# OpenPPL/ppl.llm.serving

Measured on AMD Instinct MI355X. Metric: decode tokens/sec, LLaMA-7B int8 (W8A16), max-running-batch 1024, higher is better.
Workload: dtype fp16 activations, int8 weights (W8A16), int8-g8 KV, fp32 accumulate

## Files before the change

ppl.llm.serving_amd/csrc/k_gemm.hip:

```cpp
#include <stdarg.h>
#include <stdio.h>
#include <stdlib.h>

#include <algorithm>

#include <type_traits>
#include "k_gemm_dev.h"

namespace pplhip {

void LinearRoute::add(const char* fmt, ...) {
    if (!buf || cap <= 0 || len >= cap - 1) return;
    if (len > 0) buf[len++] = ' ';
    va_list ap;
    va_start(ap, fmt);
    const int n = vsnprintf(buf + len, (size_t)(cap - len), fmt, ap);
    va_end(ap);
    len = n < 0 ? len : (len + n < cap - 1 ? len + n : cap - 1);
    buf[len] = 0;
}

template <int WQ, int EPI>
__global__ __launch_bounds__(256) void gemm_kernel(const uint16_t* __restrict__ x, const void* __restrict__ wv,
                                                   const uint16_t* __restrict__ scale, int64_t M, int N, int K, int group,
// ... 595 lines not shown

template <class F>
void for_each_half128(F&& f) {
    f(int_c<3>{}, int_c<16>{}); f(int_c<3>{}, int_c<32>{}); f(int_c<2>{}, int_c<64>{}); f(int_c<3>{}, int_c<64>{});
    f(int_c<3>{}, int_c<80>{}); f(int_c<3>{}, int_c<96>{}); f(int_c<3>{}, int_c<112>{}); f(int_c<3>{}, int_c<128>{});
}
void run_w8_half128(const LinearPart& p, const LinearArgs& a) {
    static LdsOptIn once;
    if (once.first())
        for_each_epi([](auto E) {
            for_each_half128([&](auto ST, auto BM) { set_max_lds(half128_lds_bytes(ST, BM), gemm_w8_half128_kernel<E, ST, BM>); });
        });
    dispatch_epi(p.epi, [&](auto E) {
        for_each_half128([&](auto ST, auto BM) {
            if (ST == p.stages && BM == p.bm)
                hipLaunchKernelGGL((gemm_w8_half128_kernel<E, ST, BM>), dim3(p.grid_x, p.grid_y), dim3(p.threads), p.lds, a.s, a.x, (const int8_t*)a.w,
                                   a.scale, p.M, a.N, a.K, a.y, a.ldy, p.n_tiles, p.kt_per, a.ws);
        });
    });
}

void run_ring(const LinearPart& p, const LinearArgs& a) {
    dispatch_int<8, 4, 0>(p.wq, [&](auto WQ) {
        dispatch_epi(p.epi, [&](auto E) {
            dispatch_int<2, 3, 4>(p.stages, [&](auto ST) {
                auto go = [&](auto kernel) {
                    hipLaunchKernelGGL(kernel, dim3(p.grid_x, p.grid_y), dim3(p.threads), 0, a.s, a.x, a.w, a.scale, p.M, a.N, a.K, a.y, a.ldy, p.n_tiles,
                                       p.m_tiles, map_pack(p.map), p.kt_per, a.ws);
                };
                if constexpr (WQ == 8 && ST >= 3) {
                    if (p.wl == 6) return go(gemm_dma_kernel<WQ, E, ST, 6>);
                }
                if (p.wl == 5) go(gemm_dma_kernel<WQ, E, ST, 5>);
                else if (p.bm == 64) go(gemm_dma_kernel<WQ, E, ST, 1, 64>);
                else if (p.maxg == 16) go(gemm_dma_kernel<WQ, E, ST, 1, G_BM, 16>);
                else go(gemm_dma_kernel<WQ, E, ST, 1>);
            });
        });
    });
}

void run_generic(const LinearPart& p, const LinearArgs& a) {
    dispatch_int<0, 8, 4>(p.wq, [&](auto WQ) {
        dispatch_epi(p.epi, [&](auto E) {
            hipLaunchKernelGGL((gemm_kernel<WQ, E>), dim3(p.grid_x), dim3(p.threads), 0, a.s, a.x, a.w, a.scale, p.M, a.N, a.K, a.group, a.y, a.ldy,
                               p.n_tiles, p.m_tiles);
        });
    });
}

}

hipError_t launch_linear(hipStream_t s, const uint16_t* x, const void* w, const uint16_t* scale, int wq_bit, int group,
                         int64_t M, int N, int K, void* y, int64_t ldy, bool out_fp32, float* ws, size_t ws_bytes, bool swiglu, SplitSlabs* defer,
                         LinearRoute* route) {
    if (defer) *defer = SplitSlabs{};
    if (M == 0) return hipSuccess;
    if (swiglu && out_fp32) return hipErrorInvalidValue;
    LinearProblem pr;
    pr.wq_bit = wq_bit, pr.group = group, pr.M = M, pr.N = N, pr.K = K, pr.ldy = ldy;
    pr.epi = swiglu ? EPI_SWIGLU : (out_fp32 ? EPI_F32 : EPI_F16);
    pr.ws_bytes = ws ? ws_bytes : 0;
    pr.accept_defer = defer != nullptr;
    pr.x = (uintptr_t)x, pr.w = (uintptr_t)w, pr.scale = (uintptr_t)scale, pr.y = (uintptr_t)y;
    if (!linear_problem_valid(pr)) return hipErrorInvalidValue;
    static const LinearTuning tuning = LinearTuning::from_env();
    const LinearPlan plan = plan_linear(pr, tuning);
    if (!plan.ok) return hipErrorInvalidValue;
    if (route) {
        char text[512];
        format_route(plan, text, (int)sizeof text);
        route->add("%s", text);
        if (route->dry) return hipSuccess;
    }
    const uint16_t* rscale = wq_bit == 8 ? scale : nullptr;
    for (int i = 0; i < plan.n_parts; ++i) {
        const LinearPart& p = plan.part[i];
        const LinearArgs a{s, x + p.m0 * K, w, scale, group, N, K, (char*)y + (size_t)p.m0 * ldy * (out_fp32 ? 4 : 2), ldy, ws};
        hipError_t e = hipSuccess;
        bool sub = false;
        switch (p.family) {
            case LF_GEMV_STREAM: sub = true, e = launch_gemv_stream(s, a.x, w, scale, wq_bit, group, p.M, N, K, a.y, ldy, p.epi); break;
            case LF_W4_PC: sub = true, e = launch_linear_w4_pc(s, a.x, w, scale, p.M, N, K, a.y, ldy, p.epi); break;
            case LF_W8_WIDE: sub = true, e = launch_linear_w8_wide(s, a.x, (const int8_t*)w, scale, p.M, N, K, a.y, ldy, p.epi, p.nc); break;
            case LF_GEMV: run_gemv(p, a); break;
            case LF_W8_256: run_w8_256(p, a); break;
            case LF_W8_HALF128: run_w8_half128(p, a); break;
            case LF_RING: run_ring(p, a); break;
            case LF_GENERIC: run_generic(p, a); break;
        }
        if (!sub) e = hipGetLastError();
        if (e != hipSuccess) return e;
        if (p.reduce == LR_DEFERRED) *defer = SplitSlabs{ws, p.splits, rscale, N, p.M};
        else if (p.reduce == LR_KERNEL && (e = launch_splitk_reduce(s, ws, p.splits, p.M, N, rscale, a.y, ldy, p.epi)) != hipSuccess) return e;
    }
    return hipSuccess;
}

}
```

ppl.llm.serving_amd/csrc/k_gemm_wide.hip:

```cpp
#include <stdlib.h>
#include "k_gemm_dev.h"

namespace pplhip {

namespace {

constexpr int WD_XP = WD_XB / 1024;

template <int EPI, int ST, int NC, int ABL = 0>
__global__ __launch_bounds__((NC + WD_NP) * 64) void gemm_w8_wide_kernel(const uint16_t* __restrict__ x, const int8_t* __restrict__ w,
                                                                  const uint16_t* __restrict__ scale, int64_t M, int N, int K,
                                                                  void* __restrict__ yv, int64_t ldy, int n_tiles, int m_tiles) {
    constexpr int WD_BN = 32 * NC, WD_NC = NC;
    constexpr int WD_WB = WD_BN * G_BK, WD_WP = WD_WB / 1024;
    constexpr int WD_PP = (WD_XP + WD_WP + WD_NP - 1) / WD_NP;
    extern __shared__ __attribute__((aligned(16))) char smem_wd[];
    char* const Xs0 = smem_wd;
    char* const Wq0 = smem_wd + ST * WD_XB;

    int nt, mt;
    xcd_tile((int)blockIdx.x, m_tiles, nt, mt);
    if (nt >= n_tiles) return;
    const int n0 = nt * WD_BN;
    const int64_t m0 = (int64_t)mt * WD_BM;

    const int tid = threadIdx.x, lane = tid & 63, wave = __builtin_amdgcn_readfirstlane(tid >> 6);
    const int ktiles = K / G_BK;
    constexpr int D = ST - 1;

    if (wave >= WD_NC) {
        const int pw = wave - WD_NC;
        const char* psrc[WD_PP];
        uint32_t pdst[WD_PP];
        const uint32_t xbase = lds_addr(Xs0), wbase = lds_addr(Wq0);
        const int npc = (WD_XP + WD_WP - pw + WD_NP - 1) / WD_NP;
#pragma unroll
        for (int j = 0; j < WD_PP; ++j) {
            const int P = pw + WD_NP * j;
            if (j < WD_XP / WD_NP) {
                const int p = P * 64 + lane, row = p >> 3, pos = (p & 7) ^ ((row >> 1) & 7);
                const int c = ((pos & 3) << 1) | (pos >> 2);
                int64_t m = m0 + row;
                if (m >= M) m = M - 1;
                psrc[j] = reinterpret_cast<const char*>(x + m * K + c * 8);
                pdst[j] = __builtin_amdgcn_readfirstlane(xbase + P * 1024);
            } else {
                const int Pw = (P < WD_XP + WD_WP ? P : WD_XP) - WD_XP;
                const int p = Pw * 64 + lane, row = p >> 2, c = (p & 3) ^ w_swz(row);
                int n = n0 + row;
                if (n >= N) n = N - 1;
                psrc[j] = reinterpret_cast<const char*>(w) + (int64_t)n * K + c * 16;
                pdst[j] = __builtin_amdgcn_readfirstlane(wbase + Pw * 1024);
            }
        }
#define WD_PRODUCE(KT, STG)                                                                                                          \
    do {                                                                                                                             \
        _Pragma("unroll") for (int j = 0; j < WD_PP; ++j)                                                                            \
            if (j < npc)                                                                                                             \
            glds16(psrc[j] + (int64_t)(KT) * (j < WD_XP / WD_NP ? G_BK * 2 : G_BK), pdst[j] + (STG) * (j < WD_XP / WD_NP ? WD_XB : WD_WB)); \
    } while (0)
#pragma unroll
        for (int d = 0; d < D; ++d)
            if (d < ktiles) WD_PRODUCE(d, d);
        int stn = D % ST;
        for (int t = 0; t < ktiles; ++t) {
            const int younger = (ktiles - 1 - t) < (D - 1) ? (ktiles - 1 - t) : (D - 1);
            if (younger >= 2) {
                if (npc == WD_PP) asm volatile("s_waitcnt vmcnt(%0)" ::"n"(2 * WD_PP) : "memory");
                else asm volatile("s_waitcnt vmcnt(%0)" ::"n"(2 * WD_PP - 2) : "memory");
            } else if (younger == 1) {
                if (npc == WD_PP) asm volatile("s_waitcnt vmcnt(%0)" ::"n"(WD_PP) : "memory");
                else asm volatile("s_waitcnt vmcnt(%0)" ::"n"(WD_PP - 1) : "memory");
            } else {
                asm volatile("s_waitcnt vmcnt(0)" ::: "memory");
            }
            if (!(ABL & 8)) __syncthreads();
            if (t + D < ktiles && !(ABL & 1)) WD_PRODUCE(t + D, stn);
            stn = stn == ST - 1 ? 0 : stn + 1;
        }
#undef WD_PRODUCE
        return;
    }

    const int l15 = lane & 15, kq = lane >> 4;
    const int nb = wave * 32;
    f4 acc[2][8];
#pragma unroll
    for (int i = 0; i < 2; ++i)
#pragma unroll
        for (int j = 0; j < 8; ++j) acc[i][j] = f4{0.f, 0.f, 0.f, 0.f};
    int st = 0;
    for (int t = 0; t < ktiles; ++t) {
        if (!(ABL & 8)) __syncthreads();
        const uint16_t* xs = reinterpret_cast<const uint16_t*>(Xs0 + st * WD_XB);
        const char* wq = Wq0 + st * WD_WB;
        st = st == ST - 1 ? 0 : st + 1;
        uint4 wraw[2];
#pragma unroll
        for (int i = 0; i < 2; ++i) {
            const int row = nb + i * 16 + l15;
            wraw[i] = *reinterpret_cast<const uint4*>(&wq[row * G_BK + (kq ^ w_swz(row)) * 16]);
        }
#pragma unroll
        for (int ks = 0; ks < 2; ++ks) {
            h8 a[2], bfr[8];
#pragma unroll
            for (int i = 0; i < 2; ++i) {
                if constexpr (ABL & 2) a[i] = __builtin_bit_cast(h8, make_uint4(wraw[i].x, wraw[i].y, wraw[i].z ^ ks, wraw[i].w));
                else a[i] = cvt_i8x8_f16(ks == 0 ? make_uint2(wraw[i].x, wraw[i].y) : make_uint2(wraw[i].z, wraw[i].w));
            }
#pragma unroll
            for (int j = 0; j < 8; ++j) {
                const int row = j * 16 + l15;
                bfr[j] = __builtin_bit_cast(h8, *reinterpret_cast<const uint4*>(&xs[((ABL & 4) ? 0 : row * G_BK) + g_swz(row, ks * 4 + kq) * 8]));
            }
#pragma unroll
            for (int i = 0; i < 2; ++i)
#pragma unroll
                for (int j = 0; j < 8; ++j) acc[i][j] = __builtin_amdgcn_mfma_f32_16x16x32_f16(a[i], bfr[j], acc[i][j], 0, 0, 0);
        }
    }

#pragma unroll
    for (int i = 0; i < 2; ++i) {
        const int n = n0 + nb + i * 16 + kq * 4;
        if (n >= N) continue;
        const h4 sh = __builtin_bit_cast(h4, *reinterpret_cast<const uint2*>(scale + n));
#pragma unroll
        for (int j = 0; j < 8; ++j) {
            const int64_t m = m0 + j * 16 + l15;
            if (m >= M) continue;
            store4<EPI>(yv, ldy, m, n, acc[i][j][0] * (float)sh[0], acc[i][j][1] * (float)sh[1], acc[i][j][2] * (float)sh[2],
                        acc[i][j][3] * (float)sh[3]);
        }
    }
}

}

hipError_t launch_linear_w8_wide(hipStream_t s, const uint16_t* x, const int8_t* w, const uint16_t* scale, int64_t M, int N, int K, void* y,
                                 int64_t ldy, int epi, int nc, LinearRoute* route) {
    LinearPart p;
    if (!plan_w8_wide(M, N, epi, nc, &p)) return hipErrorInvalidValue;
    if (route_part(route, p)) return hipSuccess;
    constexpr int ST = WD_ST;
    const size_t lds = p.lds;
    const int n_tiles = p.n_tiles, m_tiles = p.m_tiles;
    static LdsOptIn once;
    if (once.first()) for_each_epi([&](auto E) { set_max_lds(lds, gemm_w8_wide_kernel<E, ST, 12>); });
    dim3 grid(p.grid_x);
#ifdef WD_ABLATE_BUILD
    static const int abl = getenv("PPLHIP_GEMM_WIDE_ABLATE") ? atoi(getenv("PPLHIP_GEMM_WIDE_ABLATE")) : 0;
    bool ablated = true;
    dispatch_int<1, 2, 3, 4, 6, 7, 8, 15, 0>(abl, [&](auto A) {
        if constexpr (A == 0) ablated = false;
        else {
            set_max_lds(lds, gemm_w8_wide_kernel<EPI_F16, ST, 12, A>);
            hipLaunchKernelGGL((gemm_w8_wide_kernel<EPI_F16, ST, 12, A>), grid, dim3((12 + WD_NP) * 64), lds, s, x, w, scale, M, N, K, y, ldy, n_tiles, m_tiles);
        }
    });
    if (ablated) return hipGetLastError();
#endif
    dispatch_epi(epi, [&](auto E) {
        hipLaunchKernelGGL((gemm_w8_wide_kernel<E, ST, 12>), grid, dim3((12 + WD_NP) * 64), lds, s, x, w, scale, M, N, K, y, ldy, n_tiles, m_tiles);
    });
    return hipGetLastError();
}

}
```

ppl.llm.serving_amd/csrc/kernels.h:

```cpp
#pragma once
#include <hip/hip_runtime.h>
#include <stdint.h>
#include "k_common.h"
#include "linear_plan.h"

namespace pplhip {

struct SplitSlabs {
    const float* ws = nullptr;
    int splits = 0;
    const uint16_t* scale = nullptr;
    int N = 0;
    int64_t M = 0;
};
struct LinearRoute {
    char* buf = nullptr;
    int cap = 0;
    int len = 0;
    bool dry = false;
    void add(const char* fmt, ...) __attribute__((format(printf, 2, 3)));
};
#ifdef __HIPCC__
__device__ __forceinline__ void slab_load8(const SplitSlabs& sl, int64_t m, int n, float* o) {
    const float* p = sl.ws + m * sl.N + n;
    const int64_t zs = sl.M * sl.N;
    float4 c[8], d[8];
#pragma unroll
    for (int z = 0; z < 8; ++z) {
        const float* q = p + (z < sl.splits ? z : 0) * zs;
        c[z] = *reinterpret_cast<const float4*>(q);
        d[z] = *reinterpret_cast<const float4*>(q + 4);
    }
    float4 a = c[0], b = d[0];
#pragma unroll
    for (int z = 1; z < 8; ++z) {
        if (z < sl.splits) {
            a.x += c[z].x; a.y += c[z].y; a.z += c[z].z; a.w += c[z].w;
            b.x += d[z].x; b.y += d[z].y; b.z += d[z].z; b.w += d[z].w;
        }
    }
    if (sl.scale) {
        const h8 sh = __builtin_bit_cast(h8, *reinterpret_cast<const uint4*>(sl.scale + n));
        a.x *= (float)sh[0]; a.y *= (float)sh[1]; a.z *= (float)sh[2]; a.w *= (float)sh[3];
        b.x *= (float)sh[4]; b.y *= (float)sh[5]; b.z *= (float)sh[6]; b.w *= (float)sh[7];
    }
    o[0] = round_h(a.x); o[1] = round_h(a.y); o[2] = round_h(a.z); o[3] = round_h(a.w);
    o[4] = round_h(b.x); o[5] = round_h(b.y); o[6] = round_h(b.z); o[7] = round_h(b.w);
}
#endif

hipError_t launch_embedding(hipStream_t s, const int64_t* token_ids, const uint16_t* table, int64_t T, int hidden,
                            uint16_t* out);
hipError_t launch_rmsnorm(hipStream_t s, const uint16_t* x, const uint16_t* skip, const uint16_t* w, float eps,
                          int64_t rows, int hidden, const int64_t* gather_seq_starts, uint16_t* out,
                          uint16_t* residual_out, int8_t* qout = nullptr, float* sx = nullptr,
                          const SplitSlabs* skip_slabs = nullptr,
                          bool q_fp8 = false);
struct RmsnormForm {
    int maxc = 0, nt = 0;
};
hipError_t rmsnorm_form(int64_t rows, int hidden, int wide_max_rows, RmsnormForm* f);
int rmsnorm_wide_max_rows();
hipError_t launch_silu_mul(hipStream_t s, const uint16_t* gate_up, int64_t T, int inter, uint16_t* out);
hipError_t launch_gather_last_rows(hipStream_t s, const uint16_t* x, const int64_t* seq_starts, int64_t B, int hidden, uint16_t* out);

hipError_t launch_rope_kv_write(hipStream_t s, uint16_t* qkv, const float* cos_sin, const KvAddr& kv, int kv_fmt,
                                const int64_t* seq_starts, const int64_t* start_pos,
                                const int64_t* cache_indices, int64_t max_pages, int64_t B, int64_t t0, int64_t T, int H,
                                int Hkv, int D, const SplitSlabs* qkv_slabs = nullptr);

size_t attn_decode_workspace_bytes(int64_t nb, int H, int D, int split);
hipError_t launch_attn_decode(hipStream_t s, const uint16_t* qkv, const KvAddr& kv, int kv_fmt,
                              const int64_t* seq_starts, const int64_t* start_pos, const int64_t* cache_indices,
                              int64_t max_pages, int64_t nb, int H, int Hkv, int D, int64_t max_kv_len, int split,
                              int threads, float* workspace, uint16_t* out, hipEvent_t t0 = nullptr, hipEvent_t t1 = nullptr);
hipError_t launch_attn_reduce(hipStream_t s, const float* ws, int nsplit, int64_t n_row_heads, int D, uint16_t* out);

hipError_t launch_attn_prefill(hipStream_t s, const uint16_t* qkv, const KvAddr& kv, int kv_fmt,
                               const int64_t* seq_starts, const int64_t* start_pos, const int64_t* cache_indices,
                               int64_t max_pages, int64_t b0, int64_t B, int H, int Hkv, int D, int64_t max_seq_len,
                               uint16_t* out, int64_t max_kv_len = 0, float* ws = nullptr, size_t ws_bytes = 0, int64_t row0 = 0,
                               int64_t nrows = 0);

hipError_t launch_attn_prefill32(hipStream_t s, const uint16_t* qkv, const KvAddr& kv, int kv_fmt, const int64_t* seq_starts,
                                 const int64_t* start_pos, const int64_t* cache_indices, int64_t max_pages, int64_t b0, int64_t B,
                                 int H, int Hkv, int D, int64_t max_seq_len, uint16_t* out, int64_t max_kv_len = 0, float* ws = nullptr,
                                 size_t ws_bytes = 0, int64_t row0 = 0, int64_t nrows = 0);

bool attn_decode_gqa_supported(int kv_fmt, int H, int Hkv, int D);
hipError_t launch_attn_decode_gqa(hipStream_t s, const uint16_t* qkv, const KvAddr& kv, int kv_fmt,
                                  const int64_t* seq_starts, const int64_t* start_pos, const int64_t* cache_indices,
                                  int64_t max_pages, int64_t nb, int H, int Hkv, int D, int split, float* workspace,
                                  uint16_t* out, hipEvent_t t0 = nullptr, hipEvent_t t1 = nullptr);

hipError_t launch_linear_w8_wide(hipStream_t s, const uint16_t* x, const int8_t* w, const uint16_t* scale, int64_t M, int N, int K, void* y,
                                 int64_t ldy, int epi, int nc, LinearRoute* route = nullptr);
hipError_t launch_linear_w4_pc(hipStream_t s, const uint16_t* x, const void* w, const uint16_t* scale, int64_t M, int N, int K, void* y,
                               int64_t ldy, int epi, LinearRoute* route = nullptr);
hipError_t launch_linear(hipStream_t s, const uint16_t* x, const void* w, const uint16_t* scale, int wq_bit, int group,
                         int64_t M, int N, int K, void* y, int64_t ldy, bool out_fp32, float* ws = nullptr, size_t ws_bytes = 0,
                         bool swiglu = false, SplitSlabs* defer = nullptr,
                         LinearRoute* route = nullptr);
hipError_t launch_splitk_reduce(hipStream_t s, const float* ws, int splits, int64_t M, int N, const uint16_t* scale, void* y, int64_t ldy, int epi);
hipError_t launch_gemv_stream(hipStream_t s, const uint16_t* x, const void* w, const uint16_t* scale, int wq_bit, int group, int64_t M, int N,
                              int K, void* y, int64_t ldy, int epi, LinearRoute* route = nullptr);
hipError_t launch_quant_act(hipStream_t s, const uint16_t* x, int64_t M, int K, int64_t ldx, int8_t* q, int64_t ldq, float* sx);
hipError_t launch_quant_weight(hipStream_t s, const uint16_t* w, int N, int K, int8_t* q, int64_t ldq, uint16_t* scale);
hipError_t launch_linear_i8(hipStream_t s, const int8_t* xq, const float* sx, const int8_t* w, const uint16_t* scale, int64_t M, int N,
                            int K, void* y, int64_t ldy, bool out_fp32, bool swiglu);
hipError_t launch_quant_act_f8(hipStream_t s, const uint16_t* x, int64_t M, int K, int64_t ldx, uint8_t* q, int64_t ldq, float* sx);
hipError_t launch_quant_weight_f8(hipStream_t s, const uint16_t* w, int N, int K, uint8_t* q, int64_t ldq, uint16_t* scale);
hipError_t launch_linear_f8(hipStream_t s, const uint8_t* xq, const float* sx, const uint8_t* w, const uint16_t* scale, int64_t M, int N,
                            int K, void* y, int64_t ldy, bool out_fp32, bool swiglu);
hipError_t launch_interleave_rows(hipStream_t s, const void* src, void* dst, int rows, int64_t row_bytes);

constexpr int LORA_MAX_SLOTS = 64, LORA_MAX_RANK = 128;
struct LoraTile {
    int32_t slot;
    int32_t n;
    int32_t row[16];
};
struct LoraSlot {
    const uint16_t* a;
    const uint16_t* b;
    int32_t rp;
    float scale;
};
hipError_t launch_lora(hipStream_t s, const LoraTile* tiles, int ntiles, const LoraSlot* slots, const uint16_t* x, int64_t ldx, uint16_t* y,
                       int64_t ldy, int N, int K, uint16_t* t);

constexpr int P2P_MAX_RANKS = 8;
constexpr int P2P_MAX_BLOCKS = 64;
constexpr size_t P2P_FLAGS_START = 0;
constexpr size_t P2P_FLAGS_MID = (size_t)P2P_MAX_BLOCKS * P2P_MAX_RANKS * 4;
constexpr int P2P_CHANNELS = 2;
constexpr size_t P2P_CHANNEL_FLAG_BYTES = (size_t)2 * P2P_MAX_BLOCKS * P2P_MAX_RANKS * 4;
constexpr size_t P2P_DATA_START = 8192;
static_assert(P2P_CHANNELS * P2P_CHANNEL_FLAG_BYTES <= P2P_DATA_START, "flag words of every channel in front of the data");
constexpr uint32_t P2P_FLAG_REFRESH_EPOCHS = 1u << 30;
struct P2pPeers {
    char* base[P2P_MAX_RANKS];
};
hipError_t launch_p2p_flag_refresh(hipStream_t s, char* my_base, int channel, uint32_t epoch);
hipError_t launch_p2p_allreduce(hipStream_t s, const P2pPeers& peers, int me, int n, size_t data_off, size_t scratch_off, int64_t count,
                                uint32_t epoch, uint64_t timeout_ticks, uint32_t* status, int channel = 0);
constexpr int P2P_NORM_MAX_HIDDEN = 8192;
hipError_t launch_p2p_allreduce_norm(hipStream_t s, const P2pPeers& peers, int me, int n, size_t data_off, size_t scratch_off, int64_t rows,
                                     int hidden, uint16_t* h, const uint16_t* w, float eps, uint16_t* xn, uint32_t epoch, uint64_t timeout_ticks,
                                     uint32_t* status, int channel = 0);
hipError_t launch_p2p_allgather(hipStream_t s, const P2pPeers& peers, int me, int n, size_t src_off, void* dst, int64_t rows,
                                int64_t row_bytes, int64_t dst_row_bytes, uint32_t epoch, uint64_t timeout_ticks, uint32_t* status);

hipError_t launch_handoff_signal(hipStream_t s, uint32_t* flag, uint32_t epoch);
hipError_t launch_handoff_wait(hipStream_t s, const uint32_t* wait_flag, uint32_t wait_epoch, uint32_t* done_flag, uint32_t done_epoch,
                               uint64_t timeout_ticks, uint32_t* status);

float p2p_pattern_value(int64_t i, int g, int round);
hipError_t launch_p2p_pattern(hipStream_t s, uint16_t* halfs, int64_t cnt, float* floats, int64_t gcnt, int g, int round);

hipError_t launch_sample_greedy(hipStream_t s, const float* logits, const float* temperatures, int batch, int vocab,
                                int stride, int32_t* out_tok, float* out_logprob);
size_t sample_topk_workspace_bytes(int batch, int vocab, int top_k);
hipError_t launch_sample_topk_topp(hipStream_t s, const float* logits, const float* temperatures, const float* top_p,
                                   const float* rnd, int batch, int vocab, int stride, int top_k, float default_top_p,
                                   void* workspace, int32_t* out_tok, float* out_logprob);
hipError_t launch_penalty(hipStream_t s, float* logits, const float* temperatures, const float* rep,
                          const float* presence, const float* frequency, const int64_t* batch_slots,
                          const int64_t* token_inputs, const int64_t* seq_starts, const int64_t* start_pos, int batch,
                          int vocab, int stride, int decoding_batches, uint16_t* count_map);

hipError_t launch_sample_rows(hipStream_t s, const float* logits, const float* temperatures, const int32_t* top_k, const float* top_p,
                              const uint64_t* seeds, const uint64_t* draws, const float* rnd, const int32_t* rows, int n_greedy,
                              int n_sampling, int vocab, int stride, int32_t* out_tok, float* out_logprob);
hipError_t launch_sample_uniform(hipStream_t s, const uint64_t* seeds, const uint64_t* draws, int batch, float* out_u);

constexpr int TOP_LOGPROBS_MAX = 20;
hipError_t launch_top_logprobs(hipStream_t s, const float* logits, const float* temperatures, const int32_t* num_logprobs,
                               const int32_t* rows, int n_rows, int vocab, int stride, int32_t* out_tok, float* out_logprob);

// ... 41 lines not shown
```

ppl.llm.serving_amd/csrc/linear_plan.cc:

```cpp
#include "linear_plan.h"

#include <stdio.h>
#include <stdlib.h>

#include "k_tune.h"

namespace pplhip {

LinearTuning LinearTuning::from_env() {
    LinearTuning t;
    t.msplit = tune_int("PPLHIP_GEMM_MSPLIT", t.msplit);
    t.no_skinny = tune_set("PPLHIP_GEMM_NOSKINNY");
    t.force_generic = tune_set("PPLHIP_GEMM_GENERIC");
    t.gemv_max_m = tune_int("PPLHIP_GEMV_MAX_M", t.gemv_max_m);
    t.gemv_max_m_set = tune_set("PPLHIP_GEMV_MAX_M");
    if (const char* v = getenv("PPLHIP_GEMV_STREAM_MAX_M")) t.gemv_stream_max_m = atoi(v);
    t.gemv_waves = tune_int("PPLHIP_GEMV_WAVES", t.gemv_waves);
    if (const char* v = getenv("PPLHIP_GEMM_PC")) t.pc_mode = atoi(v);
    t.wide = tune_int("PPLHIP_GEMM_WIDE", t.wide);
    t.min_m256 = tune_int("PPLHIP_GEMM_256_MIN_M", t.min_m256);
    t.gm256 = tune_int("PPLHIP_GEMM256_GM", t.gm256);
    t.gn256 = tune_int("PPLHIP_GEMM256_GN", t.gn256);
    t.direct_epilogue = tune_set("PPLHIP_GEMM_DIRECT_EPILOGUE");
    t.map = tune_int("PPLHIP_GEMM_MAP", t.map);
    t.gm128_set = tune_set("PPLHIP_GEMM128_GM");
    t.gm128 = tune_int("PPLHIP_GEMM128_GM", t.gm128);
    t.gn128 = tune_int("PPLHIP_GEMM128_GN", t.gn128);
    t.ablate = tune_int("PPLHIP_GEMM_ABLATE", t.ablate);
    t.stages = tune_int("PPLHIP_GEMM_STAGES", t.stages);
    t.splitk = tune_int("PPLHIP_GEMM_SPLITK", t.splitk);
    t.minkt = tune_int("PPLHIP_GEMM_MINKT", t.minkt);
    t.split_deep = tune_int("PPLHIP_GEMM_SPLIT_DEEP", t.split_deep);
    t.wl = tune_int("PPLHIP_GEMM_WL", t.wl);
    t.half = tune_int("PPLHIP_GEMM_HALF", t.half);
    t.half128 = tune_int("PPLHIP_GEMM_HALF128", t.half128);
    t.half128_max_m = tune_int("PPLHIP_GEMM_HALF128_MAX_M", t.half128_max_m);
    t.half128_blocks = tune_int("PPLHIP_GEMM_HALF128_BLOCKS", t.half128_blocks);
    t.half128_unsplit_max_m = tune_int("PPLHIP_GEMM_HALF128_UNSPLIT_MAX_M", t.half128_unsplit_max_m);
    t.w4_sc16 = tune_int("PPLHIP_GEMM_W4_SC16", t.w4_sc16);
    return t;
}

int gemv_stream_max_m(int wq_bit, int group, int N, int K, int env_max_m) {
    const int max_m = env_max_m >= 0 ? env_max_m : (wq_bit == 8 && K % 128 == 0 ? 2 : 4);
    const int kl = wq_bit == 8 ? 16 : (wq_bit == 4 ? 32 : 8);
    if (K % kl) return 0;
    if (wq_bit == 4 && (group % 32 || K % group)) return 0;
    const int pieces = (K / kl + 63) / 64;
    if (pieces > 3 * GV_NW) return 0;
    (void)N;
    return max_m > 4 ? 4 : max_m;
}

int linear_w8_wide_waves(int64_t M, int N) {
    const int64_t m_tiles = (M + WD_BM - 1) / WD_BM;
    const int64_t tiles = (N + 383) / 384 * m_tiles, rounds = (tiles + 255) / 256;
    const double eff = (double)N * (double)M / ((double)rounds * 256.0 * 384.0 * WD_BM);
    return (eff >= 0.85 && (rounds <= 2 || eff >= 0.97)) ? 12 : 0;
}

bool linear_w4_pc_supported(int group, int64_t M, int N, int K, uintptr_t x, uintptr_t w, uintptr_t scale, uintptr_t y, int64_t ldy, int epi) {
    if (group != 128 || K % 128 || K < 128 || N % 4 || M < 1) return false;
    if (epi != EPI_F16 && epi != EPI_SWIGLU) return false;
    if (epi == EPI_SWIGLU && N % 16) return false;
    if (ldy % 8 || (y & 15)) return false;
    if ((x & 15) || (w & 15) || (scale & 3)) return false;
    if ((uint64_t)M * (uint64_t)K * 2 >= (1ull << 32) || (uint64_t)N * (uint64_t)K / 2 >= (1ull << 32)) return false;
    if ((uint64_t)N * (uint64_t)(K / 128) >= (1ull << 30)) return false;
    return true;
}

static unsigned xcd_grid(int n_tiles, int m_tiles) { return (unsigned)((n_tiles + 7) / 8 * 8 * m_tiles); }

bool plan_gemv_stream(int wq_bit, int64_t M, int N, int K, int epi, LinearPart* p) {
    const int kl = wq_bit == 8 ? 16 : (wq_bit == 4 ? 32 : 8);
    const int pieces = (K / kl + 63) / 64;
    int nwk_log2 = 0;
    while ((1 << nwk_log2) < pieces && nwk_log2 < 3) ++nwk_log2;
    const int nwk = 1 << nwk_log2, npw = (pieces + nwk - 1) / nwk;
    const int nw = nwk <= 4 ? 4 : 8;
    const int64_t waves16 = (int64_t)((N + 15) / 16) * nwk;
    const int nb = waves16 >= 2048 ? 2 : 1;
    const int rows = (nw / nwk) * nb * GV_U;
    if (M < 1 || M > 4 || npw > 3) return false;
    if (wq_bit != 8 && wq_bit != 4 && wq_bit != 0) return false;
    p->family = LF_GEMV_STREAM;
    p->M = M, p->wq = wq_bit, p->epi = epi, p->nw = nw;
    p->bn = rows, p->bm = 4;
    p->n_tiles = (N + rows - 1) / rows, p->m_tiles = 1;
    p->grid_x = (unsigned)p->n_tiles, p->threads = (unsigned)nw * 64;
    p->nwk_log2 = nwk_log2, p->npw = npw, p->nb = nb;
    return true;
}

bool plan_w4_pc(int64_t M, int N, int epi, LinearPart* p) {
    p->family = LF_W4_PC;
    p->M = M, p->wq = 4, p->epi = epi;
    p->bn = PC_BN, p->bm = PC_BM;
    p->n_tiles = (N + PC_BN - 1) / PC_BN, p->m_tiles = (int)((M + PC_BM - 1) / PC_BM);
    p->grid_x = xcd_grid(p->n_tiles, p->m_tiles), p->threads = 512, p->lds = PC_LDS;
    return true;
}

bool plan_w8_wide(int64_t M, int N, int epi, int nc, LinearPart* p) {
    if (nc != 12) return false;
    p->family = LF_W8_WIDE;
    p->M = M, p->wq = 8, p->epi = epi, p->stages = WD_ST, p->nc = nc;
    p->bn = 32 * nc, p->bm = WD_BM;
    p->n_tiles = (N + p->bn - 1) / p->bn, p->m_tiles = (int)((M + WD_BM - 1) / WD_BM);
    p->grid_x = xcd_grid(p->n_tiles, p->m_tiles), p->threads = (unsigned)(nc + WD_NP) * 64, p->lds = (size_t)wide_lds_bytes(WD_ST, nc);
    return true;
}

static bool plan_part(const LinearProblem& pr, const LinearTuning& t, int64_t m0, int64_t M, bool defer, LinearPart* p) {
    const int wq = pr.wq_bit, group = pr.group, N = pr.N, K = pr.K, epi = pr.epi;
    const bool ws = pr.ws_bytes > 0;
    const size_t ws_bytes = pr.ws_bytes;
    const uintptr_t x = pr.x + (uintptr_t)(m0 * K * 2), y = pr.y + (uintptr_t)(m0 * pr.ldy * (epi == EPI_F32 ? 4 : 2));
    *p = LinearPart{};
    p->M = M, p->wq = wq, p->epi = epi;
    bool ok = true;
    if (M <= gemv_stream_max_m(wq, group, N, K, t.gemv_stream_max_m) && !t.no_skinny && !t.force_generic) {
        ok = plan_gemv_stream(wq, M, N, K, epi, p);
    } else if (M <= (ws ? (wq == 8 && K % (G_BK * 2) == 0 && t.gemv_max_m > 2 && !t.gemv_max_m_set ? 2 : t.gemv_max_m) : 16) && M <= 16 && !t.no_skinny) {
        p->family = LF_GEMV;
        p->nw = (t.gemv_waves ? t.gemv_waves : ((N + 15) / 16 <= 1024 ? 8 : 4)) == 8 ? 8 : 4;
        p->bn = 16, p->bm = 16;
        p->n_tiles = (N + 15) / 16, p->m_tiles = 1;
        p->grid_x = (unsigned)p->n_tiles, p->threads = (unsigned)p->nw * 64;
    } else if (t.pc_mode && wq == 4 && M > 128 && M <= 512 && !t.force_generic && (int64_t)((N + 63) / 64) * ((M + 127) / 128) >= 160 &&
               linear_w4_pc_supported(group, M, N, K, x, pr.w, pr.scale, y, pr.ldy, epi)) {
        ok = plan_w4_pc(M, N, epi, p);
    } else if (t.wide && wq == 8 && K % G_BK == 0 && M >= 512 && (M < 4096 || t.wide == 2) && N >= 8192 &&
               (t.wide == 2 || linear_w8_wide_waves(M, N) == 12)) {
        ok = plan_w8_wide(M, N, epi, 12, p);
    } else {
        const int n_tiles = (N + G_BN - 1) / G_BN, m_tiles = (int)((M + G_BM - 1) / G_BM);
        const bool w4_fast = wq == 4 && group == 128 && K % 128 == 0 &&
                             (K / 128 <= W4_MAXG || (ws && (size_t)((K / 128 + W4_MAXG - 1) / W4_MAXG) * M * N * sizeof(float) <= ws_bytes));
        p->n_tiles = n_tiles, p->m_tiles = m_tiles;
        p->bn = G_BN, p->bm = G_BM;
        if (wq == 8 && K % G_BK == 0 && M >= t.min_m256 && N >= 1024 && !t.force_generic) {
            const int nt2 = (N + H_BN - 1) / H_BN, mt2 = (int)((M + H_BM - 1) / H_BM);
            const int nl = (nt2 + 7) / 8;
            int gm = t.gm256 > 0 && t.gm256 <= 255 ? t.gm256 : 4;
            while (gm > 1 && mt2 % gm) --gm;
            int gn = t.gn256 > 0 && t.gn256 <= 255 ? t.gn256 : 8;
            if (gn > nl) gn = nl;
            p->family = LF_W8_256;
            p->bn = H_BN, p->bm = H_BM, p->stages = H_ST;
            p->n_tiles = nt2, p->m_tiles = mt2;
            p->map = MapMode{0, 0, (uint8_t)gm, (uint8_t)gn};
            p->grid_x = (unsigned)(8 * ((nl + gn - 1) / gn * gn) * mt2), p->threads = 512, p->lds = H_LDS;
            p->staged = !t.direct_epilogue && pr.ldy % 8 == 0 && (y & 15) == 0 && (epi != EPI_SWIGLU || N % 16 == 0) ? 1 : 0;
        } else if ((wq == 8 || wq == 0 || w4_fast) && K % G_BK == 0 && !t.force_generic) {
            const int64_t tiles = (int64_t)n_tiles * m_tiles;
            const bool st_forced = t.stages >= 2 && t.stages <= 4;
            int stages = st_forced ? t.stages : (tiles <= 256 ? 4 : 2);
            if (wq == 0 && stages == 4) stages = 3;
            const int kt_all = K / G_BK;
            int splits = 1;
            if (ws && ((M <= 256 && tiles < 512) || tiles < 200 || t.splitk > 0)) {
                const int target = M <= 64 ? 768 : 512;
                splits = (int)((target + tiles - 1) / tiles);
                const int cap = (M <= 64 || tiles <= 32) ? 8 : 4;
                if (splits > cap) splits = cap;
                if (M > 64 && tiles >= 160) splits = 1;
                const int min_kt = t.minkt ? t.minkt : ((M <= 64 || tiles <= 64) ? 16 : 28);
                if (splits > kt_all / min_kt) splits = kt_all / min_kt > 0 ? kt_all / min_kt : 1;
                if (t.splitk > 0) splits = t.splitk;
                while (splits > 1 && (size_t)splits * M * N * sizeof(float) > ws_bytes) --splits;
            }
            if (wq == 4 && splits < (kt_all + 2 * W4_MAXG - 1) / (2 * W4_MAXG)) splits = (kt_all + 2 * W4_MAXG - 1) / (2 * W4_MAXG);
            int kt_per = (kt_all + splits - 1) / splits;
            if (wq == 4) kt_per = (kt_per + 1) & ~1;
            splits = (kt_all + kt_per - 1) / kt_per;
            if (splits > 1 && !st_forced) stages = (t.split_deep && tiles * splits <= 256 && !(wq == 4 && M <= 64)) ? (wq == 0 ? 3 : 4) : 2;
            int wl = (t.wl == 1 || t.wl == 5) ? t.wl : (tiles * splits <= 256 ? 5 : 1);
            const bool half = t.half >= 0 ? (t.half == 1 && M <= 64) : M <= 64;
            if (half) wl = 1;
            if ((t.wl == 6 || (t.wl == 0 && wl == 5)) && wq == 8 && stages >= 3 && splits == 1) wl = 6;
            int sp = splits;
            const int kt128 = K / (G_BK * S_KS);
            if (ws && t.splitk <= 0) {
                sp = t.half128_blocks / n_tiles;
                if (sp > 8) sp = 8;
                if (sp < 1) sp = 1;
                while (sp > 1 && (size_t)sp * M * N * sizeof(float) > ws_bytes) --sp;
            }
            if (sp > kt128) sp = kt128 > 0 ? kt128 : 1;
            if (t.half128 && (half || (M <= 128 && M <= t.half128_max_m && (sp > 1 || M <= t.half128_unsplit_max_m) && m_tiles == 1)) && wq == 8 &&
                K % (G_BK * S_KS) == 0) {
                const int kt_per128 = (kt128 + sp - 1) / sp;
                sp = (kt128 + kt_per128 - 1) / kt_per128;
                const int bm = M > 64 ? (int)((M + 15) / 16 * 16) : (t.half128 == 2 ? 64 : (M <= 16 ? 16 : (M <= 32 ? 32 : 64)));
                p->family = LF_W8_HALF128;
                p->bm = bm, p->stages = (bm <= 32 || bm > 64 || (int64_t)n_tiles * sp <= 256) ? 3 : 2;
                p->splits = sp, p->kt_per = kt_per128, p->kt_depth = G_BK * S_KS;
                p->grid_x = (unsigned)n_tiles, p->grid_y = (unsigned)sp, p->threads = 256, p->lds = (size_t)half128_lds_bytes(p->stages, bm);
            } else {
                const bool w4_small_sc = t.w4_sc16 && wq == 4 && splits > 1 && kt_per <= 32 && wl == 1 && !half && stages == 2;
                p->family = LF_RING;
                p->stages = stages, p->wl = 1, p->bm = G_BM, p->maxg = W4_MAXG;
                if (wl == 6 && wq == 8 && stages >= 3) p->wl = 6;
                else if (wl == 5) p->wl = 5;
                else if (half) p->bm = 64;
                else if (w4_small_sc) p->maxg = 16;
                p->splits = splits, p->kt_per = kt_per, p->kt_depth = G_BK;
                p->threads = p->wl == 6 ? 768 : (p->wl == 5 ? 512 : 256);
                p->grid_x = xcd_grid(n_tiles, m_tiles), p->grid_y = (unsigned)splits;
                p->map.ablate = (uint8_t)t.ablate;
                if (t.map == 1 && m_tiles % 8 == 0) {
                    p->map.order = 1;
                    p->grid_x = (unsigned)(n_tiles * m_tiles);
                } else if (m_tiles > 8 || t.gm128_set) {
                    int gm = t.gm128 > 0 ? t.gm128 : 8;
                    while (gm > 1 && m_tiles % gm) --gm;
                    const int nl = (n_tiles + 7) / 8;
// ... 83 lines not shown
```

ppl.llm.serving_amd/csrc/linear_plan.h:

```cpp
#pragma once
#include <stddef.h>
#include <stdint.h>

#include "k_gemm_tiles.h"

namespace pplhip {

struct LinearTuning {
    int msplit = 256;
    bool no_skinny = false;
    bool force_generic = false;
    int gemv_max_m = 3;
    bool gemv_max_m_set = false;
    int gemv_stream_max_m = -1;
    int gemv_waves = 0;
    int pc_mode = 1;
    int wide = 1;
    int min_m256 = 3584;
    int gm256 = 0, gn256 = 0;
    bool direct_epilogue = false;
    int map = -1;
    bool gm128_set = false;
    int gm128 = 0, gn128 = 0;
    int ablate = 0;
    int stages = 0;
    int splitk = 0;
    int minkt = 0;
    int split_deep = 1;
    int wl = 0;
    int half = -1;
    int half128 = 1;
    int half128_max_m = 128;
    int half128_blocks = 256;
    int half128_unsplit_max_m = 80;
    int w4_sc16 = 1;
    static LinearTuning from_env();
};

struct LinearProblem {
    int wq_bit = 0, group = 0;
    int64_t M = 0;
    int N = 0, K = 0;
    int64_t ldy = 0;
    int epi = EPI_F16;
    size_t ws_bytes = 0;
    bool accept_defer = false;
    uintptr_t x = 0, w = 0, scale = 0, y = 0;
};

enum LinearFamily { LF_GEMV_STREAM, LF_GEMV, LF_W4_PC, LF_W8_WIDE, LF_W8_256, LF_W8_HALF128, LF_RING, LF_GENERIC };
enum LinearReduce { LR_NONE, LR_KERNEL, LR_DEFERRED };
struct MapMode { uint8_t order, ablate, gm, gn; };
constexpr int map_pack(MapMode m) { return (int)(m.order | (unsigned)m.ablate << 8 | (unsigned)m.gm << 16 | (unsigned)m.gn << 24); }
constexpr MapMode map_unpack(int v) { return MapMode{(uint8_t)v, (uint8_t)(v >> 8), (uint8_t)(v >> 16), (uint8_t)(v >> 24)}; }

struct LinearPart {
    int64_t m0 = 0, M = 0;
    LinearFamily family = LF_GENERIC;
    int wq = 0, epi = EPI_F16, stages = 0, wl = 0, bm = 0, maxg = 0, nw = 0, nc = 0;
    unsigned grid_x = 0, grid_y = 1, threads = 0;
    size_t lds = 0;
    int bn = 0;
    int n_tiles = 0, m_tiles = 0, splits = 1, kt_per = 0, kt_depth = 0;
    MapMode map = {0, 0, 0, 0};
    int staged = 0;
    LinearReduce reduce = LR_NONE;
    int nwk_log2 = 0, npw = 0, nb = 0;
};

struct LinearPlan {
    bool ok = false;
    int n_parts = 0;
    LinearPart part[2];
};

bool linear_problem_valid(const LinearProblem& p);
LinearPlan plan_linear(const LinearProblem& p, const LinearTuning& t);
bool plan_gemv_stream(int wq_bit, int64_t M, int N, int K, int epi, LinearPart* part);
bool plan_w4_pc(int64_t M, int N, int epi, LinearPart* part);
bool plan_w8_wide(int64_t M, int N, int epi, int nc, LinearPart* part);

int format_route(const LinearPart& part, char* buf, int cap);
int format_route(const LinearPlan& plan, char* buf, int cap);

int gemv_stream_max_m(int wq_bit, int group, int N, int K, int env_max_m);
int linear_w8_wide_waves(int64_t M, int N);
bool linear_w4_pc_supported(int group, int64_t M, int N, int K, uintptr_t x, uintptr_t w, uintptr_t scale, uintptr_t y, int64_t ldy, int epi);

}
```

Baseline: 24040.

## Let wide W8 GEMM blocks sweep multiple N passes to balance wave quantization

Adds a multi-pass mode to the wide int8 GEMM. Each block can now cover a variable-width N span made of several 384-column passes, and consumer waves are dealt 16-column chunks so a partial final pass uses fewer waves. The planner picks a per-block column count when its cost model predicts fewer rounds than the default tiling over 256 CUs. This is meant to cut tail-round waste for large-N projections at decode batch sizes. The cost is X tiles reloaded per pass, epilogues between passes, and more complex producer indexing.

Result: no change. 24150 (median of 6 runs) (+0.4%).

```diff
diff --git a/ppl.llm.serving_amd/csrc/k_gemm.hip b/ppl.llm.serving_amd/csrc/k_gemm.hip
--- a/ppl.llm.serving_amd/csrc/k_gemm.hip
+++ b/ppl.llm.serving_amd/csrc/k_gemm.hip
@@ -701,7 +701,7 @@
         switch (p.family) {
             case LF_GEMV_STREAM: sub = true, e = launch_gemv_stream(s, a.x, w, scale, wq_bit, group, p.M, N, K, a.y, ldy, p.epi); break;
             case LF_W4_PC: sub = true, e = launch_linear_w4_pc(s, a.x, w, scale, p.M, N, K, a.y, ldy, p.epi); break;
-            case LF_W8_WIDE: sub = true, e = launch_linear_w8_wide(s, a.x, (const int8_t*)w, scale, p.M, N, K, a.y, ldy, p.epi, p.nc); break;
+            case LF_W8_WIDE: sub = true, e = launch_linear_w8_wide(s, a.x, (const int8_t*)w, scale, p.M, N, K, a.y, ldy, p.epi, p.nc, tuning.wide_passes); break;
             case LF_GEMV: run_gemv(p, a); break;
             case LF_W8_256: run_w8_256(p, a); break;
             case LF_W8_HALF128: run_w8_half128(p, a); break;
diff --git a/ppl.llm.serving_amd/csrc/k_gemm_wide.hip b/ppl.llm.serving_amd/csrc/k_gemm_wide.hip
--- a/ppl.llm.serving_amd/csrc/k_gemm_wide.hip
+++ b/ppl.llm.serving_amd/csrc/k_gemm_wide.hip
@@ -10,10 +10,12 @@
 template <int EPI, int ST, int NC, int ABL = 0>
 __global__ __launch_bounds__((NC + WD_NP) * 64) void gemm_w8_wide_kernel(const uint16_t* __restrict__ x, const int8_t* __restrict__ w,
                                                                   const uint16_t* __restrict__ scale, int64_t M, int N, int K,
-                                                                  void* __restrict__ yv, int64_t ldy, int n_tiles, int m_tiles) {
+                                                                  void* __restrict__ yv, int64_t ldy, int n_tiles, int m_tiles, int bn) {
     constexpr int WD_BN = 32 * NC, WD_NC = NC;
+    constexpr int WD_CH = WD_BN / 16;
     constexpr int WD_WB = WD_BN * G_BK, WD_WP = WD_WB / 1024;
     constexpr int WD_PP = (WD_XP + WD_WP + WD_NP - 1) / WD_NP;
+    static_assert(NC % 4 == 0, "the chunk deal: quads of consumer waves");
     extern __shared__ __attribute__((aligned(16))) char smem_wd[];
     char* const Xs0 = smem_wd;
     char* const Wq0 = smem_wd + ST * WD_XB;
@@ -21,11 +23,15 @@
     int nt, mt;
     xcd_tile((int)blockIdx.x, m_tiles, nt, mt);
     if (nt >= n_tiles) return;
-    const int n0 = nt * WD_BN;
+    const int n0 = nt * bn;
     const int64_t m0 = (int64_t)mt * WD_BM;
+    const int cleft = (N + 15) / 16 - nt * (bn >> 4);
+    const int cb = cleft < (bn >> 4) ? cleft : (bn >> 4);
+    const int npass = (cb + WD_CH - 1) / WD_CH;
 
     const int tid = threadIdx.x, lane = tid & 63, wave = __builtin_amdgcn_readfirstlane(tid >> 6);
     const int ktiles = K / G_BK;
+    const int steps = npass * ktiles;
     constexpr int D = ST - 1;
 
     if (wave >= WD_NC) {
@@ -34,6 +40,7 @@
         uint32_t pdst[WD_PP];
         const uint32_t xbase = lds_addr(Xs0), wbase = lds_addr(Wq0);
         const int npc = (WD_XP + WD_WP - pw + WD_NP - 1) / WD_NP;
+        const int nlast = (n0 + cb * 16 < N ? n0 + cb * 16 : N) - 1;
 #pragma unroll
         for (int j = 0; j < WD_PP; ++j) {
             const int P = pw + WD_NP * j;
@@ -46,25 +53,42 @@
                 pdst[j] = __builtin_amdgcn_readfirstlane(xbase + P * 1024);
             } else {
                 const int Pw = (P < WD_XP + WD_WP ? P : WD_XP) - WD_XP;
-                const int p = Pw * 64 + lane, row = p >> 2, c = (p & 3) ^ w_swz(row);
-                int n = n0 + row;
-                if (n >= N) n = N - 1;
-                psrc[j] = reinterpret_cast<const char*>(w) + (int64_t)n * K + c * 16;
                 pdst[j] = __builtin_amdgcn_readfirstlane(wbase + Pw * 1024);
             }
         }
+#define WD_WEIGHT_SRC(PASS)                                                                                                          \
+    do {                                                                                                                             \
+        _Pragma("unroll") for (int j = WD_XP / WD_NP; j < WD_PP; ++j) {                                                              \
+            const int P = pw + WD_NP * j;                                                                                            \
+            const int Pw = (P < WD_XP + WD_WP ? P : WD_XP) - WD_XP;                                                                  \
+            const int p = Pw * 64 + lane, row = p >> 2, c = (p & 3) ^ w_swz(row);                                                    \
+            int n = n0 + (PASS) * WD_BN + row;                                                                                       \
+            if (n > nlast) n = nlast;                                                                                                \
+            psrc[j] = reinterpret_cast<const char*>(w) + (int64_t)n * K + c * 16;                                                    \
+        }                                                                                                                            \
+    } while (0)
 #define WD_PRODUCE(KT, STG)                                                                                                          \
     do {                                                                                                                             \
         _Pragma("unroll") for (int j = 0; j < WD_PP; ++j)                                                                            \
             if (j < npc)                                                                                                             \
             glds16(psrc[j] + (int64_t)(KT) * (j < WD_XP / WD_NP ? G_BK * 2 : G_BK), pdst[j] + (STG) * (j < WD_XP / WD_NP ? WD_XB : WD_WB)); \
     } while (0)
+#define WD_ISSUE_NEXT()                                                                                                              \
+    do {                                                                                                                             \
+        WD_PRODUCE(ik, stn);                                                                                                         \
+        stn = stn == ST - 1 ? 0 : stn + 1;                                                                                           \
+        if (++ik == ktiles) {                                                                                                        \
+            ik = 0, ++ip;                                                                                                            \
+            WD_WEIGHT_SRC(ip);                                                                                                       \
+        }                                                                                                                            \
+    } while (0)
+        int ik = 0, ip = 0, stn = 0;
+        WD_WEIGHT_SRC(0);
 #pragma unroll
         for (int d = 0; d < D; ++d)
-            if (d < ktiles) WD_PRODUCE(d, d);
-        int stn = D % ST;
-        for (int t = 0; t < ktiles; ++t) {
-            const int younger = (ktiles - 1 - t) < (D - 1) ? (ktiles - 1 - t) : (D - 1);
+            if (d < steps) WD_ISSUE_NEXT();
+        for (int g = 0; g < steps; ++g) {
+            const int younger = (steps - 1 - g) < (D - 1) ? (steps - 1 - g) : (D - 1);
             if (younger >= 2) {
                 if (npc == WD_PP) asm volatile("s_waitcnt vmcnt(%0)" ::"n"(2 * WD_PP) : "memory");
                 else asm volatile("s_waitcnt vmcnt(%0)" ::"n"(2 * WD_PP - 2) : "memory");
@@ -75,77 +99,101 @@
                 asm volatile("s_waitcnt vmcnt(0)" ::: "memory");
             }
             if (!(ABL & 8)) __syncthreads();
-            if (t + D < ktiles && !(ABL & 1)) WD_PRODUCE(t + D, stn);
-            stn = stn == ST - 1 ? 0 : stn + 1;
-        }
+            if (g + D < steps && !(ABL & 1)) WD_ISSUE_NEXT();
+        }
+#undef WD_ISSUE_NEXT
 #undef WD_PRODUCE
+#undef WD_WEIGHT_SRC
         return;
     }
 
     const int l15 = lane & 15, kq = lane >> 4;
-    const int nb = wave * 32;
+    const int kb = (wave & 3) + 8 * (wave >> 2);
     f4 acc[2][8];
-#pragma unroll
-    for (int i = 0; i < 2; ++i)
-#pragma unroll
-        for (int j = 0; j < 8; ++j) acc[i][j] = f4{0.f, 0.f, 0.f, 0.f};
     int st = 0;
-    for (int t = 0; t < ktiles; ++t) {
-        if (!(ABL & 8)) __syncthreads();
-        const uint16_t* xs = reinterpret_cast<const uint16_t*>(Xs0 + st * WD_XB);
-        const char* wq = Wq0 + st * WD_WB;
-        st = st == ST - 1 ? 0 : st + 1;
-        uint4 wraw[2];
+    auto k_loop = [&](auto NS) {
+        for (int t = 0; t < ktiles; ++t) {
+            if (!(ABL & 8)) asm volatile("s_waitcnt lgkmcnt(0)\n\ts_barrier" ::: "memory");
+            const uint16_t* xs = reinterpret_cast<const uint16_t*>(Xs0 + st * WD_XB);
+            const char* wq = Wq0 + st * WD_WB;
+            st = st == ST - 1 ? 0 : st + 1;
+            if constexpr (NS > 0) {
+                uint4 wraw[NS];
+#pragma unroll
+                for (int i = 0; i < NS; ++i) {
+                    const int row = (kb + 4 * i) * 16 + l15;
+                    wraw[i] = *reinterpret_cast<const uint4*>(&wq[row * G_BK + (kq ^ w_swz(row)) * 16]);
+                }
+#pragma unroll
+                for (int ks = 0; ks < 2; ++ks) {
+                    h8 a[NS], bfr[8];
+#pragma unroll
+                    for (int i = 0; i < NS; ++i) {
+                        if constexpr (ABL & 2) a[i] = __builtin_bit_cast(h8, make_uint4(wraw[i].x, wraw[i].y, wraw[i].z ^ ks, wraw[i].w));
+                        else a[i] = cvt_i8x8_f16(ks == 0 ? make_uint2(wraw[i].x, wraw[i].y) : make_uint2(wraw[i].z, wraw[i].w));
+                    }
+#pragma unroll
+                    for (int j = 0; j < 8; ++j) {
+                        const int row = j * 16 + l15;
+                        bfr[j] = __builtin_bit_cast(h8, *reinterpret_cast<const uint4*>(&xs[((ABL & 4) ? 0 : row * G_BK) + g_swz(row, ks * 4 + kq) * 8]));
+                    }
+#pragma unroll
+                    for (int i = 0; i < NS; ++i)
+#pragma unroll
+                        for (int j = 0; j < 8; ++j) acc[i][j] = __builtin_amdgcn_mfma_f32_16x16x32_f16(a[i], bfr[j], acc[i][j], 0, 0, 0);
+                }
+            }
+        }
+    };
+    for (int pass = 0; pass < npass; ++pass) {
+        const int cp = cb - pass * WD_CH;
+        const int ns = kb < cp ? (kb + 4 < cp ? 2 : 1) : 0;
+#pragma unroll
+        for (int i = 0; i < 2; ++i)
+#pragma unroll
+            for (int j = 0; j < 8; ++j) acc[i][j] = f4{0.f, 0.f, 0.f, 0.f};
+        if (ns == 2) k_loop(int_c<2>{});
+        else if (ns == 1) k_loop(int_c<1>{});
+        else k_loop(int_c<0>{});
+
+        int et = tid;
+        asm volatile("" : "+v"(et));
+        const int el15 = et & 15, ekq = (et >> 4) & 3;
+        uint2 sraw[2];
+        int nn[2];
 #pragma unroll
         for (int i = 0; i < 2; ++i) {
-            const int row = nb + i * 16 + l15;
-            wraw[i] = *reinterpret_cast<const uint4*>(&wq[row * G_BK + (kq ^ w_swz(row)) * 16]);
-        }
-#pragma unroll
-        for (int ks = 0; ks < 2; ++ks) {
-            h8 a[2], bfr[8];
-#pragma unroll
-            for (int i = 0; i < 2; ++i) {
-                if constexpr (ABL & 2) a[i] = __builtin_bit_cast(h8, make_uint4(wraw[i].x, wraw[i].y, wraw[i].z ^ ks, wraw[i].w));
-                else a[i] = cvt_i8x8_f16(ks == 0 ? make_uint2(wraw[i].x, wraw[i].y) : make_uint2(wraw[i].z, wraw[i].w));
-            }
+            nn[i] = n0 + pass * WD_BN + (kb + 4 * i) * 16 + ekq * 4;
+            if (i >= ns || nn[i] >= N) nn[i] = -1;
+            sraw[i] = *reinterpret_cast<const uint2*>(scale + (nn[i] < 0 ? 0 : nn[i]));
+        }
+        asm volatile("" ::"v"(sraw[0].x), "v"(sraw[0].y), "v"(sraw[1].x), "v"(sraw[1].y));
+        const h4 sh[2] = {__builtin_bit_cast(h4, sraw[0]), __builtin_bit_cast(h4, sraw[1])};
+#pragma unroll
+        for (int i = 0; i < 2; ++i) {
+            const int n = nn[i];
+            if (n < 0) continue;
 #pragma unroll
             for (int j = 0; j < 8; ++j) {
-                const int row = j * 16 + l15;
-                bfr[j] = __builtin_bit_cast(h8, *reinterpret_cast<const uint4*>(&xs[((ABL & 4) ? 0 : row * G_BK) + g_swz(row, ks * 4 + kq) * 8]));
-            }
-#pragma unroll
-            for (int i = 0; i < 2; ++i)
-#pragma unroll
-                for (int j = 0; j < 8; ++j) acc[i][j] = __builtin_amdgcn_mfma_f32_16x16x32_f16(a[i], bfr[j], acc[i][j], 0, 0, 0);
+                const int64_t m = m0 + j * 16 + el15;
+                if (m >= M) continue;
+                store4<EPI>(yv, ldy, m, n, acc[i][j][0] * (float)sh[i][0], acc[i][j][1] * (float)sh[i][1], acc[i][j][2] * (float)sh[i][2],
+                            acc[i][j][3] * (float)sh[i][3]);
+            }
         }
     }
-
-#pragma unroll
-    for (int i = 0; i < 2; ++i) {
-        const int n = n0 + nb + i * 16 + kq * 4;
-        if (n >= N) continue;
-        const h4 sh = __builtin_bit_cast(h4, *reinterpret_cast<const uint2*>(scale + n));
-#pragma unroll
-        for (int j = 0; j < 8; ++j) {
-            const int64_t m = m0 + j * 16 + l15;
-            if (m >= M) continue;
-            store4<EPI>(yv, ldy, m, n, acc[i][j][0] * (float)sh[0], acc[i][j][1] * (float)sh[1], acc[i][j][2] * (float)sh[2],
-                        acc[i][j][3] * (float)sh[3]);
-        }
-    }
 }
 
 }
 
 hipError_t launch_linear_w8_wide(hipStream_t s, const uint16_t* x, const int8_t* w, const uint16_t* scale, int64_t M, int N, int K, void* y,
-                                 int64_t ldy, int epi, int nc, LinearRoute* route) {
+                                 int64_t ldy, int epi, int nc, int passes, LinearRoute* route) {
     LinearPart p;
-    if (!plan_w8_wide(M, N, epi, nc, &p)) return hipErrorInvalidValue;
+    if (!plan_w8_wide(M, N, epi, nc, passes, &p)) return hipErrorInvalidValue;
     if (route_part(route, p)) return hipSuccess;
     constexpr int ST = WD_ST;
     const size_t lds = p.lds;
-    const int n_tiles = p.n_tiles, m_tiles = p.m_tiles;
+    const int n_tiles = p.n_tiles, m_tiles = p.m_tiles, bn = p.bn;
     static LdsOptIn once;
     if (once.first()) for_each_epi([&](auto E) { set_max_lds(lds, gemm_w8_wide_kernel<E, ST, 12>); });
     dim3 grid(p.grid_x);
@@ -156,13 +204,13 @@
         if constexpr (A == 0) ablated = false;
         else {
             set_max_lds(lds, gemm_w8_wide_kernel<EPI_F16, ST, 12, A>);
-            hipLaunchKernelGGL((gemm_w8_wide_kernel<EPI_F16, ST, 12, A>), grid, dim3((12 + WD_NP) * 64), lds, s, x, w, scale, M, N, K, y, ldy, n_tiles, m_tiles);
+            hipLaunchKernelGGL((gemm_w8_wide_kernel<EPI_F16, ST, 12, A>), grid, dim3((12 + WD_NP) * 64), lds, s, x, w, scale, M, N, K, y, ldy, n_tiles, m_tiles, bn);
         }
     });
     if (ablated) return hipGetLastError();
 #endif
     dispatch_epi(epi, [&](auto E) {
-        hipLaunchKernelGGL((gemm_w8_wide_kernel<E, ST, 12>), grid, dim3((12 + WD_NP) * 64), lds, s, x, w, scale, M, N, K, y, ldy, n_tiles, m_tiles);
+        hipLaunchKernelGGL((gemm_w8_wide_kernel<E, ST, 12>), grid, dim3((12 + WD_NP) * 64), lds, s, x, w, scale, M, N, K, y, ldy, n_tiles, m_tiles, bn);
     });
     return hipGetLastError();
 }
diff --git a/ppl.llm.serving_amd/csrc/kernels.h b/ppl.llm.serving_amd/csrc/kernels.h
--- a/ppl.llm.serving_amd/csrc/kernels.h
+++ b/ppl.llm.serving_amd/csrc/kernels.h
@@ -94,7 +94,7 @@
                                   uint16_t* out, hipEvent_t t0 = nullptr, hipEvent_t t1 = nullptr);
 
 hipError_t launch_linear_w8_wide(hipStream_t s, const uint16_t* x, const int8_t* w, const uint16_t* scale, int64_t M, int N, int K, void* y,
-                                 int64_t ldy, int epi, int nc, LinearRoute* route = nullptr);
+                                 int64_t ldy, int epi, int nc, int passes, LinearRoute* route = nullptr);
 hipError_t launch_linear_w4_pc(hipStream_t s, const uint16_t* x, const void* w, const uint16_t* scale, int64_t M, int N, int K, void* y,
                                int64_t ldy, int epi, LinearRoute* route = nullptr);
 hipError_t launch_linear(hipStream_t s, const uint16_t* x, const void* w, const uint16_t* scale, int wq_bit, int group,
diff --git a/ppl.llm.serving_amd/csrc/linear_plan.cc b/ppl.llm.serving_amd/csrc/linear_plan.cc
--- a/ppl.llm.serving_amd/csrc/linear_plan.cc
+++ b/ppl.llm.serving_amd/csrc/linear_plan.cc
@@ -17,6 +17,7 @@
     if (const char* v = getenv("PPLHIP_GEMV_STREAM_MAX_M")) t.gemv_stream_max_m = atoi(v);
     t.gemv_waves = tune_int("PPLHIP_GEMV_WAVES", t.gemv_waves);
     if (const char* v = getenv("PPLHIP_GEMM_PC")) t.pc_mode = atoi(v);
+    if (const char* v = getenv("PPLHIP_GEMM_WIDE_PASSES")) t.wide_passes = atoi(v);
     t.wide = tune_int("PPLHIP_GEMM_WIDE", t.wide);
     t.min_m256 = tune_int("PPLHIP_GEMM_256_MIN_M", t.min_m256);
     t.gm256 = tune_int("PPLHIP_GEMM256_GM", t.gm256);
@@ -102,12 +103,20 @@
     return true;
 }
 
-bool plan_w8_wide(int64_t M, int N, int epi, int nc, LinearPart* p) {
+static int wide_pass_cost(int c) { return 6 * (c / 24) + (c % 24 + 3) / 4; }
+
+bool plan_w8_wide(int64_t M, int N, int epi, int nc, int passes, LinearPart* p) {
     if (nc != 12) return false;
     p->family = LF_W8_WIDE;
     p->M = M, p->wq = 8, p->epi = epi, p->stages = WD_ST, p->nc = nc;
     p->bn = 32 * nc, p->bm = WD_BM;
     p->n_tiles = (N + p->bn - 1) / p->bn, p->m_tiles = (int)((M + WD_BM - 1) / WD_BM);
+    const int64_t rounds = ((int64_t)p->n_tiles * p->m_tiles + 255) / 256;
+    const int G = p->m_tiles <= 32 ? 256 / p->m_tiles / 8 * 8 : 0, C = (N + 15) / 16;
+    if (passes && G > 0) {
+        const int c = (C + G - 1) / G;
+        if (wide_pass_cost(c) < 6 * rounds) p->bn = 16 * c, p->n_tiles = (C + c - 1) / c;
+    }
     p->grid_x = xcd_grid(p->n_tiles, p->m_tiles), p->threads = (unsigned)(nc + WD_NP) * 64, p->lds = (size_t)wide_lds_bytes(WD_ST, nc);
     return true;
 }
@@ -133,7 +142,7 @@
         ok = plan_w4_pc(M, N, epi, p);
     } else if (t.wide && wq == 8 && K % G_BK == 0 && M >= 512 && (M < 4096 || t.wide == 2) && N >= 8192 &&
                (t.wide == 2 || linear_w8_wide_waves(M, N) == 12)) {
-        ok = plan_w8_wide(M, N, epi, 12, p);
+        ok = plan_w8_wide(M, N, epi, 12, t.wide_passes, p);
     } else {
         const int n_tiles = (N + G_BN - 1) / G_BN, m_tiles = (int)((M + G_BM - 1) / G_BM);
         const bool w4_fast = wq == 4 && group == 128 && K % 128 == 0 &&
diff --git a/ppl.llm.serving_amd/csrc/linear_plan.h b/ppl.llm.serving_amd/csrc/linear_plan.h
--- a/ppl.llm.serving_amd/csrc/linear_plan.h
+++ b/ppl.llm.serving_amd/csrc/linear_plan.h
@@ -16,6 +16,7 @@
     int gemv_waves = 0;
     int pc_mode = 1;
     int wide = 1;
+    int wide_passes = 1;
     int min_m256 = 3584;
     int gm256 = 0, gn256 = 0;
     bool direct_epilogue = false;
@@ -78,7 +79,7 @@
 LinearPlan plan_linear(const LinearProblem& p, const LinearTuning& t);
 bool plan_gemv_stream(int wq_bit, int64_t M, int N, int K, int epi, LinearPart* part);
 bool plan_w4_pc(int64_t M, int N, int epi, LinearPart* part);
-bool plan_w8_wide(int64_t M, int N, int epi, int nc, LinearPart* part);
+bool plan_w8_wide(int64_t M, int N, int epi, int nc, int passes, LinearPart* part);
 
 int format_route(const LinearPart& part, char* buf, int cap);
 int format_route(const LinearPlan& plan, char* buf, int cap);
```
